# mad-red/VSR-guided-CIC

Measured on AMD Instinct MI355X. Metric: decoded tokens/sec at batch=100, beam=5, 36x2048 regions, higher is better.
Workload: dtype f16x2; 1 GPU; beam-5 decode, batch 100 images/GPU, 36 regions x 2048-d, 10 slots, seq_len 20, vocab 10000 (BASELINE configs[2]); beam=5, batch_per_gpu=100, seq_len=20, parallelism=images sharded, dp1, no data-path collective, rccl_world_size_observed=1, collective_backend=nccl

## Files before the change

### vsr-guided-cic_amd/csrc/kernels.h

```cpp
#pragma once
#include <hip/hip_runtime.h>
#include <stdint.h>

namespace vsr {

constexpr int KMAX = 8;

__device__ __forceinline__ float slab_sum(const float* __restrict__ p, int nslab, long long stride, float init = 0.f) {
    float v[8];
#pragma unroll
    for (int k = 0; k < 8; ++k) v[k] = k < nslab ? p[k * stride] : 0.f;
    float s = init;
#pragma unroll
    for (int k = 0; k < 8; ++k)
        if (k < nslab) s += v[k];
    return s;
}

__device__ __forceinline__ float sigmoidf_(float x) { return 1.0f / (1.0f + expf(-x)); }

__device__ __forceinline__ uint16_t bf16_bits(float x) {
    typedef __bf16 b2 __attribute__((ext_vector_type(2)));
    typedef float f2 __attribute__((ext_vector_type(2)));
    const f2 v = {x, 0.f};
    return (uint16_t)(__builtin_bit_cast(uint32_t, __builtin_convertvector(v, b2)) & 0xffffu);
}
__device__ __forceinline__ uint2 bf16_bits4(float4 v) {
    typedef __bf16 b2 __attribute__((ext_vector_type(2)));
    typedef float f2 __attribute__((ext_vector_type(2)));
    const f2 lo = {v.x, v.y}, hi = {v.z, v.w};
    return make_uint2(__builtin_bit_cast(uint32_t, __builtin_convertvector(lo, b2)), __builtin_bit_cast(uint32_t, __builtin_convertvector(hi, b2)));
}

__device__ __forceinline__ void img_store(uint16_t* __restrict__ img, long long idx, float v, float isc) {
    if (isc == 0.f) { img[idx] = bf16_bits(v); return; }
    const float x = v * isc;
    const _Float16 hi = (_Float16)x;
    const _Float16 lo = (_Float16)(x - (float)hi);
    uint16_t* g = img + ((idx >> 3) << 4) + (idx & 7);
    g[0] = __builtin_bit_cast(uint16_t, hi);
    g[8] = __builtin_bit_cast(uint16_t, lo);
}
__device__ __forceinline__ void img_store4(uint16_t* __restrict__ img, long long idx , float4 v, float isc) {
    if (isc == 0.f) { *reinterpret_cast<uint2*>(img + idx) = bf16_bits4(v); return; }
    typedef _Float16 h4 __attribute__((ext_vector_type(4)));
    typedef float f4 __attribute__((ext_vector_type(4)));
    const f4 x = {v.x * isc, v.y * isc, v.z * isc, v.w * isc};
    const h4 hi = __builtin_convertvector(x, h4);
    const f4 rr = x - __builtin_convertvector(hi, f4);
    const h4 lo = __builtin_convertvector(rr, h4);
    uint16_t* g = img + ((idx >> 3) << 4) + (idx & 7);
    *reinterpret_cast<uint2*>(g) = __builtin_bit_cast(uint2, hi);
    *reinterpret_cast<uint2*>(g + 8) = __builtin_bit_cast(uint2, lo);
}

__device__ __forceinline__ float wave_sum(float v) {
#pragma unroll
    for (int o = 32; o > 0; o >>= 1) v += __shfl_xor(v, o, 64);
    return v;
}
__device__ __forceinline__ float wave_max(float v) {
#pragma unroll
    for (int o = 32; o > 0; o >>= 1) v = fmaxf(v, __shfl_xor(v, o, 64));
    return v;
}

__device__ __forceinline__ int xcd_item(int n) {
    const int chunk = (n + 7) >> 3;
    const int it = (blockIdx.x & 7) * chunk + (blockIdx.x >> 3);
    return it < n ? it : -1;
}

__global__ __launch_bounds__(256) void k_pool(const float* __restrict__ det, const int* __restrict__ row_img,
                                              const float* __restrict__ dmask, int R0, int D, float* __restrict__ vbar) {
    const int b = blockIdx.x, d = (blockIdx.y * 256 + threadIdx.x) * 4;
    const int img = row_img ? row_img[b] : b;
    const float* X = det + (long long)img * R0 * D;
    const float* mk = dmask + (long long)img * R0;
    float n = 0.f;
    for (int r = 0; r < R0; ++r) n += mk[r];
    if (d >= D) return;
    float4 s = make_float4(0.f, 0.f, 0.f, 0.f);
    for (int r = 0; r < R0; ++r) {
        const float4 v = *reinterpret_cast<const float4*>(X + (long long)r * D + d);
        s.x += v.x; s.y += v.y; s.z += v.z; s.w += v.w;
    }
    *reinterpret_cast<float4*>(vbar + (long long)b * D + d) = make_float4(s.x / n, s.y / n, s.z / n, s.w / n);
}

__global__ __launch_bounds__(256) void k_rowmask(const float* __restrict__ X, long long rows, int D, float* __restrict__ mask,
                                                 float* __restrict__ blockmax = nullptr) {
    const long long row = (long long)blockIdx.x * 4 + (threadIdx.x >> 6);
    const int lane = threadIdx.x & 63;
    float s = 0.f, mx = 0.f;
    if (row < rows) {
        for (int d = lane * 4; d < D; d += 256) {
            float4 v = *reinterpret_cast<const float4*>(X + row * D + d);
            s += (v.x + v.y) + (v.z + v.w);
            if (blockmax) mx = fmaxf(fmaxf(mx, fmaxf(fabsf(v.x), fabsf(v.y))), fmaxf(fabsf(v.z), fabsf(v.w)));
        }
        s = wave_sum(s);
        if (lane == 0) mask[row] = (s != 0.f) ? 1.f : 0.f;
    }
    if (blockmax) {
        __shared__ float wm[4];
        mx = wave_max(mx);
        if (lane == 0) wm[threadIdx.x >> 6] = mx;
        __syncthreads();
        if (threadIdx.x == 0) blockmax[blockIdx.x] = fmaxf(fmaxf(wm[0], wm[1]), fmaxf(wm[2], wm[3]));
    }
}
__global__ __launch_bounds__(1024) void k_max_reduce(const float* __restrict__ v, long long n, unsigned* __restrict__ out) {
    __shared__ float wm[16];
    float m = 0.f;
    bool nan = false;
    for (long long i = threadIdx.x; i < n; i += 1024) { const float x = v[i]; nan |= !(x == x); m = fmaxf(m, x); }
    if (nan) m = __int_as_float(0x7f800000);
    m = wave_max(m);
    if ((threadIdx.x & 63) == 0) wm[threadIdx.x >> 6] = m;
    __syncthreads();
    if (threadIdx.x == 0) {
        for (int w = 1; w < 16; ++w) m = fmaxf(m, wm[w]);
        *out = __float_as_uint(m);
    }
}

__global__ void k_index_rows(const int* __restrict__ slot_idx, const int* __restrict__ row_img, const float* __restrict__ bmask,
                             int B, int LR, int Rb, int n_img, int* __restrict__ ridx, float* __restrict__ rmask,
                             int* __restrict__ bad) {
    const long long i = (long long)blockIdx.x * blockDim.x + threadIdx.x;
    if (i >= (long long)B * LR) return;
    const int b = (int)(i / LR);
    const int img = row_img ? row_img[b] : b;
    const int id = slot_idx[i];
    int row = -1;
    if (id >= Rb || id < -1 || img < 0 || img >= n_img) atomicAdd(bad, 1);
    else if (id >= 0) row = img * Rb + id;
    ridx[i] = row;
    rmask[i] = row >= 0 ? bmask[row] : 0.f;
}

__global__ __launch_bounds__(64) void k_reorder_slots(const int* __restrict__ slot_in, const int* __restrict__ rank,
                                                      const float* __restrict__ verbs_in, const float* __restrict__ bmask,
                                                      const int* __restrict__ row_img, int L, int R, int Rb,
                                                      int* __restrict__ slot_out, float* __restrict__ verbs_out) {
    extern __shared__ int sh[];
    int* src = sh;
// ... 16 lines not shown
    }
    __syncthreads();
    for (int i = tid; i < L * R; i += 64) {
        const int j = i / R, r = i - j * R;
        slot_out[(long long)n * L * R + i] = src[j] >= 0 ? S[src[j] * R + r] : -1;
    }
    if (verbs_in)
        for (int j = tid; j < L; j += 64) {
            const int rk = rank[(long long)n * L + j];
            verbs_out[(long long)n * L + j] = (rk >= 0 && rk < L) ? verbs_in[(long long)n * L + rk] : -1.f;
        }
}

__global__ __launch_bounds__(256) void k_compact_count(const float* __restrict__ mask, int rows, int* __restrict__ bcount) {
    __shared__ int wsum[4];
    const int r = blockIdx.x * 256 + threadIdx.x;
    const bool v = r < rows && mask[r] != 0.f;
    const int n = __popcll(__ballot(v));
    if ((threadIdx.x & 63) == 0) wsum[threadIdx.x >> 6] = n;
    __syncthreads();
    if (threadIdx.x == 0) bcount[blockIdx.x] = wsum[0] + wsum[1] + wsum[2] + wsum[3];
}

__global__ __launch_bounds__(1024) void k_compact_scan(int* __restrict__ bcount, int nblocks, int* __restrict__ total) {
    __shared__ int part[1024];
    const int tid = threadIdx.x;
    const int per = (nblocks + 1023) / 1024;
    const int b0 = tid * per, b1 = min(nblocks, b0 + per);
    int n = 0;
    for (int b = b0; b < b1; ++b) n += bcount[b];
    part[tid] = n;
    __syncthreads();
    for (int o = 1; o < 1024; o <<= 1) {
        const int v = tid >= o ? part[tid - o] : 0;
        __syncthreads();
        part[tid] += v;
        __syncthreads();
    }
    int run = part[tid] - n;
    for (int b = b0; b < b1; ++b) { const int c = bcount[b]; bcount[b] = run; run += c; }
    if (tid == 1023) *total = part[1023];
}

__global__ __launch_bounds__(256) void k_compact_write(const float* __restrict__ mask, int rows, const int* __restrict__ boffset,
                                                       int* __restrict__ vlist) {
    __shared__ int wsum[4];
    const int r = blockIdx.x * 256 + threadIdx.x, lane = threadIdx.x & 63, wave = threadIdx.x >> 6;
    const bool v = r < rows && mask[r] != 0.f;
    const unsigned long long bal = __ballot(v);
    if (lane == 0) wsum[wave] = __popcll(bal);
    __syncthreads();
    int base = boffset[blockIdx.x];
    for (int w = 0; w < wave; ++w) base += wsum[w];
    if (v) vlist[base + __popcll(bal & ((1ull << lane) - 1ull))] = r;
}

__global__ void k_pad_row_list(int* __restrict__ vlist, int* __restrict__ counts, int bound) {
    const int i = blockIdx.x * blockDim.x + threadIdx.x;
    const int n = counts[0];
    if (i == 0) {
        if (n > bound) counts[3] = n - bound;
        if (counts[1] != 0) atomicAdd(counts + 2, counts[1]);
    }
    if (i >= n && i < bound) vlist[i] = n > 0 ? vlist[0] : 0;
}

__global__ void k_zero_rows_beyond(const int* __restrict__ vlist, const int* __restrict__ counts, int bound, int A, float* __restrict__ P) {
    const int n = counts[0];
    for (int i = bound + (int)blockIdx.x; i < n; i += (int)gridDim.x) {
        float* row = P + (long long)vlist[i] * A;
        for (int a = threadIdx.x; a < A; a += blockDim.x) row[a] = 0.f;
    }
}

__global__ void k_slab_reduce_scatter(const float* __restrict__ slabs, int nslab, long long stride, int rows, int A,
                                      const int* __restrict__ vlist, float* __restrict__ P, const int* __restrict__ rows_dev = nullptr) {
    const long long i = (long long)blockIdx.x * blockDim.x + threadIdx.x;
    if (rows_dev && *rows_dev < rows) rows = *rows_dev;
    if (i >= (long long)rows * A) return;
    const int m = (int)(i / A), a = (int)(i % A);
    float s = slab_sum(slabs + i, nslab, stride);
    P[(long long)vlist[m] * A + a] = s;
}

__global__ void k_vproj_finish(const float* __restrict__ slabs, int nsplit, long long stride, int B, int H,
                               const float* b_ih, const float* b_hh, const float* b_is, const float* b_hs,
                               const float* b_ig, const float* b_hg, float* __restrict__ out) {
    const long long i = (long long)blockIdx.x * blockDim.x + threadIdx.x;
    const int N = 6 * H;
    if (i >= (long long)B * N) return;
    const int n = (int)(i % N);
    float s = slab_sum(slabs + i, nsplit, stride);
    float bias;
    if (n < 4 * H) bias = b_ih[n] + b_hh[n];
    else if (n < 5 * H) bias = b_is[n - 4 * H] + b_hs[n - 4 * H];
    else bias = b_ig[n - 5 * H] + b_hg[n - 5 * H];
    out[i] = s + bias;
}

__global__ void k_slab_reduce(const float* __restrict__ slabs, int nsplit, long long stride, long long n, float* __restrict__ out) {
    const long long i = (long long)blockIdx.x * blockDim.x + threadIdx.x;
    if (i >= n) return;
    float s = slab_sum(slabs + i, nsplit, stride);
    out[i] = s;
}

__global__ void k_init_rows(int* __restrict__ slot, int* __restrict__ word, int bos, int n) {
    const int i = blockIdx.x * blockDim.x + threadIdx.x;
    if (i < n) { slot[i] = 0; word[i] = bos; }
}

__global__ void k_count_outside_unit(const float* __restrict__ x, long long n, int* __restrict__ count) {
    const long long i = (long long)blockIdx.x * blockDim.x + threadIdx.x;
    const bool bad = i < n && !(fabsf(x[i]) < 1.9990234375f);
    const unsigned long long b = __ballot(bad);
    if ((threadIdx.x & 63) == 0 && b) atomicAdd(count, __popcll(b));
}

__global__ void k_fill_i32(int* p, int v, int n) {
    const int i = blockIdx.x * blockDim.x + threadIdx.x;
    if (i < n) p[i] = v;
}
__global__ void k_i64_to_i32(const int64_t* src, long long src_stride, int* dst, int n, int hi, int* __restrict__ bad) {
    const int i = blockIdx.x * blockDim.x + threadIdx.x;
    if (i >= n) return;
    long long v = src[(long long)i * src_stride];
    if (v < 0 || v >= hi) {
        atomicAdd(bad, 1);
        v = v < 0 ? 0 : hi - 1;
    }
    dst[i] = (int)v;
}
__global__ void k_i32_to_i64(const int* src, int64_t* dst, int n) {
    const int i = blockIdx.x * blockDim.x + threadIdx.x;
    if (i < n) dst[i] = src[i];
}

__device__ __forceinline__ void lstm1_point(const float (&q)[6], float c_old, long long i, float* __restrict__ h1n, float* __restrict__ c1n,
                                            float* __restrict__ s_t, float* __restrict__ gpre, uint16_t* __restrict__ h1n16,
                                            uint16_t* __restrict__ s_t16, float isc) {
    const float c = sigmoidf_(q[1]) * c_old + sigmoidf_(q[0]) * tanhf(q[2]);
    const float tc = tanhf(c);
    const float h1v = sigmoidf_(q[3]) * tc, stv = sigmoidf_(q[4]) * tc;
    h1n[i] = h1v;
    c1n[i] = c;
    s_t[i] = stv;
    gpre[i] = q[5];
    if (h1n16) { img_store(h1n16, i, h1v, isc); img_store(s_t16, i, stv, isc); }
}

__global__ void k_lstm1(const float* __restrict__ pre, int nsplit, long long stride, const float* __restrict__ vproj,
                        int rpi, const int* __restrict__ parent, const float* __restrict__ c1_old, int M, int H,
                        float* __restrict__ h1n, float* __restrict__ c1n, float* __restrict__ s_t, float* __restrict__ gpre,
                        const float* __restrict__ xproj, const int* __restrict__ word, int nblk, int pre_by_parent,
                        uint16_t* __restrict__ h1n16, uint16_t* __restrict__ s_t16 , float isc = 0.f,
                        int skip5 = 0 ) {
    const long long i = (long long)blockIdx.x * blockDim.x + threadIdx.x;
    if (i >= (long long)M * H) return;
    const int row = (int)(i / H), j = (int)(i % H);
    const int prow = parent ? parent[row] : row;
    const long long base = (long long)(pre_by_parent ? prow : row) * 6 * H + j;
    const float* vp = vproj + (long long)(row / rpi) * 6 * H + j;
    const float* xp = xproj ? xproj + (long long)word[row] * 6 * H + j : nullptr;
    float q[6];
#pragma unroll
    for (int g = 0; g < 6; ++g) {
        const int sk = g == 5 ? skip5 : 0;
        float s = g < nblk ? slab_sum(pre + base + (long long)g * H + sk * stride, nsplit - sk, stride) : 0.f;
        if (xp) s += xp[(long long)g * H];
        q[g] = s + vp[(long long)g * H];
    }
// ... 834 lines not shown
            const float co = c1_old[(long long)(b * cb + wave) * H + j];
#pragma unroll
            for (int g = 0; g < 6; ++g) {
                const int sk = g == 5 ? skip5 : 0;
                sums[(wave * 7 + g) * SL_UB + u] = g < nblk ? slab_sum(pre + base + (long long)g * H + sk * stride, nsplit - sk, stride) : 0.f;
            }
            sums[(wave * 7 + 6) * SL_UB + u] = co;
        }
    }
    __syncthreads();
    if (wave == K || j >= H) return;
    const int pl = sel_s[wave], w = sel_s[KMAX + wave];
    const int row = b * K + wave;
    const float* xp = xproj + (long long)w * 6 * H + j;
    float q[6];
#pragma unroll
    for (int g = 0; g < 6; ++g) {
        float s = sums[(pl * 7 + g) * SL_UB + u];
        s += xp[(long long)g * H];
        q[g] = s + vp[g];
    }
    lstm1_point(q, sums[(pl * 7 + 6) * SL_UB + u], (long long)row * H + j, h1n, c1n, s_t, gpre, h1n16, s_t16, isc);
}

__global__ __launch_bounds__(64) void k_backtrack(int T, int B, int beam, int out_size, const float* __restrict__ seq,
                                                  const int* __restrict__ hist_parent, const int* __restrict__ hist_word,
                                                  const int* __restrict__ hist_gate, const float* __restrict__ hist_lpw,
                                                  const float* __restrict__ hist_lpg, int64_t* __restrict__ words, int64_t* __restrict__ gates,
                                                  float* __restrict__ lp_w, float* __restrict__ lp_g, float* __restrict__ scores) {
    extern __shared__ int bt[];
    const int b = blockIdx.x, lane = threadIdx.x;
    const int n = T * beam;
    int* par = bt;
    int* wrd = bt + n;
    int* gat = bt + 2 * n;
    for (int i = lane; i < n; i += 64) {
        const int t = i / beam, q = i - t * beam;
        const long long hrow = (long long)t * B * beam + b * beam + q;
        par[i] = hist_parent[hrow];
        wrd[i] = hist_word[hrow];
        gat[i] = hist_gate[hrow];
    }
    __shared__ int order[KMAX];
    if (lane == 0) {
        for (int q = 0; q < beam; ++q) order[q] = q;
        for (int a = 1; a < beam; ++a) {
// ... 29 lines not shown
```

### vsr-guided-cic_amd/csrc/vsrcap.hip

```cpp
#include "../../include/vsrcap.h"

#include <hip/hip_runtime.h>

#include <algorithm>
#include <cstdarg>
#include <cstdio>
#include <cstdlib>
#include <cstring>
#include <vector>

#include "gemm_route.h"
#include "step_gemms.h"
#include "kernels.h"
#include "train_kernels.h"

using namespace vsr;

static thread_local char g_err[512] = "";
static int fail(const char* fmt, ...) {
    va_list ap;
    va_start(ap, fmt);
    vsnprintf(g_err, sizeof(g_err), fmt, ap);
    va_end(ap);
    return 1;
// ... 380 lines not shown

static const size_t H2_HEAD = 4096;
constexpr int H2_NDYN = 512;
static_assert(H2_DYN0 * 4 + H2_NDYN * 4 <= 4096, "dynamic slots inside the head");
extern "C" size_t vsr_h2_weight_bytes(const vsr_handle* h) {
    if (!h) return 0;
    const float* p[B16_NW]; size_t n[B16_NW];
    vsr_weights none;
    memset(&none, 0, sizeof(none));
    b16_weight_list(h->d, none, p, n);
    size_t tot = H2_HEAD;
    for (int i = 0; i < B16_NW; ++i) tot += ((n[i] + 7) & ~size_t(7)) * sizeof(float);
    tot += (((size_t)h->d.vocab_size * h->d.input_encoding_size + 7) & ~size_t(7)) * sizeof(float);
    return tot + 256;
}
__global__ void k_h2_head_init(int* exps, unsigned* bounds, int* idx) {
    const int i = threadIdx.x;
    if (i < H2_NSLOT) {
        exps[i] = 0;
        bounds[i] = i == H2A_UNIT ? __float_as_uint(1.f) : 0u;
        idx[i] = i; idx[H2_NSLOT + i] = -1; idx[2 * H2_NSLOT + i] = i;
    }
}
__global__ void k_h2_prepare_exps(const unsigned* __restrict__ bounds, int R0, int* __restrict__ exps) {
    if (threadIdx.x != 0) return;
    const float r = __uint_as_float(bounds[H2A_REGION]), dt = __uint_as_float(bounds[H2A_DET]), sn = __uint_as_float(bounds[H2B_SENT]);
    exps[H2A_REGION] = h2_exp_of(r);
    exps[H2A_DET] = h2_exp_of(dt * (float)R0);
    exps[H2A_ATT] = h2_exp_of(fmaxf(r, sn));
}
extern "C" int vsr_refresh_h2_weights(vsr_handle* h, void* buffer, size_t bytes, void* stream) {
    if (!h) return fail("vsr_refresh_h2_weights: null handle");
    if (!buffer) {
        if (h->h2_on) void_derived(h, VOID_FLAVOUR);
        h->h2_on = false;
        h->h2.clear(); h->h2t.clear();
        return 0;
    }
    if (!h->bound) return fail("vsr_refresh_h2_weights: weights not bound");
    const vsr_dims& d = h->d;
    if (d.det_feat_size % 8 || d.input_encoding_size % 8 || d.rnn_size % 8 || d.att_size % 8)
        return fail("vsr_refresh_h2_weights: the f16x2 flavour needs det_feat_size, input_encoding_size, rnn_size and att_size to be "
                    "multiples of 8 (whole 8-element groups of the fp16-pair images); got %d %d %d %d", d.det_feat_size, d.input_encoding_size, d.rnn_size, d.att_size);
    if (bytes < vsr_h2_weight_bytes(h)) return fail("vsr_refresh_h2_weights: buffer too small");
    if (reinterpret_cast<uintptr_t>(buffer) & 255) return fail("vsr_refresh_h2_weights: buffer must be 256-byte aligned");
    hipStream_t s = (hipStream_t)stream;
    const float* p[B16_NW]; size_t n[B16_NW];
    b16_weight_list(h->d, h->w, p, n);
    char* base = reinterpret_cast<char*>(buffer);
// ... 99 lines not shown
    hipStream_t s = (hipStream_t)stream;
    const vsr_dims& d = h->d;
    const vsr_weights& w = h->w;
    const int H = d.rnn_size, A = d.att_size, D = d.det_feat_size, E = d.input_encoding_size;
    Ctx& c = h->c;
    c.B = B; c.R0 = R0; c.L = L; c.R = R; c.beam = beam; c.Mmax = B * beam;
    c.n_img = indexed ? n_img : 0; c.Rb = indexed ? Rb : 0;
    c.det = det; c.regions = regions;
    const size_t need = carve(h, c, reinterpret_cast<char*>(workspace));
    if (need > workspace_bytes) return fail("%s: workspace too small (%zu < %zu bytes)", who, workspace_bytes, need);
    c.ridx = c.ridx_buf;
    c.rows_are_images = indexed && row_img == nullptr && n_img == B;
    h->prepared = false;
    invalidate_train_ctx(h->tc);
    drop_saved_forwards_in(h->saved, workspace, need);
    h->ws_lo = reinterpret_cast<const char*>(workspace); h->ws_bytes = need;

    const long long rows = (long long)B * L * R;
    const long long prows = indexed ? (long long)n_img * Rb : rows;
    const bool h2b = h->h2_on;
    float* bm_regions = h2b ? c.scratch : nullptr;
    float* bm_det = h2b ? c.scratch + cdiv(prows, 4) : nullptr;
    if (h2b && (size_t)(cdiv(prows, 4) + cdiv((long long)(indexed ? n_img : B) * R0, 4)) > c.scratch_floats) return fail("%s: scratch too small for the operand bounds", who);
    hipLaunchKernelGGL(k_rowmask, dim3(cdiv(prows, 4)), dim3(256), 0, s, regions, prows, D, c.bmask, bm_regions);
    HIPCHK(hipMemsetAsync(c.nvalid_dev, 0, 4 * sizeof(int), s));
    if (indexed) {
        hipLaunchKernelGGL(k_index_rows, dim3(cdiv(rows, 256)), dim3(256), 0, s, slot_idx, row_img, c.bmask, B, L * R, Rb, n_img,
                           c.ridx_buf, c.rmask, c.nvalid_dev + 1);
    }
    {
        const int nb = (int)cdiv(prows, 256);
        hipLaunchKernelGGL(k_compact_count, dim3(nb), dim3(256), 0, s, c.bmask, (int)prows, c.bcount);
        hipLaunchKernelGGL(k_compact_scan, dim3(1), dim3(1024), 0, s, c.bcount, nb, c.nvalid_dev);
        hipLaunchKernelGGL(k_compact_write, dim3(nb), dim3(256), 0, s, c.bmask, (int)prows, c.bcount, c.vlist);
    }
    LAUNCHCHK();
    const long long bound = h->rows_bound > 0 ? std::min(h->rows_bound, prows) : 0;
    int* back = nullptr;
    if (bound > 0) {
        hipLaunchKernelGGL(k_pad_row_list, dim3(cdiv(bound, 256)), dim3(256), 0, s, c.vlist, c.nvalid_dev, (int)bound);
        LAUNCHCHK();
    } else {
        if (!h->host_back) HIPCHK(hipHostMalloc(reinterpret_cast<void**>(&h->host_back), 2 * sizeof(int), hipHostMallocDefault));
        back = h->host_back;
        HIPCHK(hipMemcpyAsync(back, c.nvalid_dev, 2 * sizeof(int), hipMemcpyDeviceToHost, s));
        if (!h->ev_count) HIPCHK(hipEventCreateWithFlags(&h->ev_count, hipEventDisableTiming));
        HIPCHK(hipEventRecord(h->ev_count, s));
    }

    const long long drows = (long long)(indexed ? n_img : B) * R0;
    hipLaunchKernelGGL(k_rowmask, dim3(cdiv(drows, 4)), dim3(256), 0, s, det, drows, D, c.dmask, bm_det);
    if (h2b) {
        hipLaunchKernelGGL(k_max_reduce, dim3(1), dim3(1024), 0, s, bm_regions, (long long)cdiv(prows, 4), h->h2_bounds + H2A_REGION);
        hipLaunchKernelGGL(k_max_reduce, dim3(1), dim3(1024), 0, s, bm_det, (long long)cdiv(drows, 4), h->h2_bounds + H2A_DET);
        hipLaunchKernelGGL(k_h2_prepare_exps, dim3(1), dim3(64), 0, s, h->h2_bounds, R0, h->h2_exps);
    }
    hipLaunchKernelGGL(k_pool, dim3(B, cdiv(D, 1024)), dim3(256), 0, s, det, indexed ? row_img : nullptr, c.dmask, R0, D, c.vbar);
    LAUNCHCHK();

    const int in1 = (d.h2_first_lstm ? H : 0) + D + E;
    const int voff = d.h2_first_lstm ? H : 0;
    {
        GemmBuilder g;
        GemmProb& p0 = g.prob(B, 4 * H, c.scratch, 6 * H);
        GemmBuilder::seg(p0, c.vbar, D, nullptr, w.lstm1_weight_ih + voff, in1, D, nullptr, H2A_DET);
        GemmProb& p1 = g.prob(B, H, c.scratch + 4 * H, 6 * H);
        GemmBuilder::seg(p1, c.vbar, D, nullptr, w.W1_is_weight + voff, in1, D, nullptr, H2A_DET);
        GemmProb& p2 = g.prob(B, H, c.scratch + 5 * H, 6 * H);
        GemmBuilder::seg(p2, c.vbar, D, nullptr, w.W1_ig_weight + voff, in1, D, nullptr, H2A_DET);
        const int ns = g.finish(h);
        const long long stride = (long long)B * 6 * H;
        for (int i = 0; i < 3; ++i) g.a.p[i].slab_stride = stride;
        if (g.launch(s, h)) return fail("vproj gemm launch failed");
        const long long n = (long long)B * 6 * H;
        hipLaunchKernelGGL(k_vproj_finish, dim3(cdiv(n, 256)), dim3(256), 0, s, c.scratch, ns, stride, B, H,
                           w.lstm1_bias_ih, w.lstm1_bias_hh, w.W1_is_bias, w.W1_hs_bias, w.W1_ig_bias, w.W1_hg_bias, c.vproj);
        LAUNCHCHK();
    }
    if (d.img_second_lstm) {
        const int in2 = H + 2 * D;
// ... 8 lines not shown
        LAUNCHCHK();
    }
    c.bounded = bound > 0;
    if (bound > 0) {
        c.nvalid = (int)bound;
        if (prows > bound)
            hipLaunchKernelGGL(k_zero_rows_beyond, dim3((unsigned)std::min<long long>(prows - bound, 2048)), dim3(128), 0, s, c.vlist, c.nvalid_dev, (int)bound, A, c.P);
    } else {
        HIPCHK(hipEventSynchronize(h->ev_count));
        c.nvalid = back[0];
        if (indexed && back[1] != 0) return fail("%s: %d slot entries index outside the feature bank [-1, %d) or name an image outside [0, %d)", who, back[1], Rb, n_img);
    }
    if (c.nvalid > 0) {
        GemmBuilder g;
        g.keep_fp32 = true;
        GemmProb& p0 = g.prob(c.nvalid, A, c.scratch, A);
        GemmBuilder::seg(p0, regions, D, c.vlist, w.att_va_weight, D, D, nullptr, H2A_REGION);
        const int ns = g.finish(h);
        const long long stride = (long long)c.nvalid * A;
        if ((size_t)stride * ns > c.scratch_floats)
            return fail("%s: att_va slabs (%lld x %d floats) exceed the workspace scratch (%zu)", who, stride, ns, c.scratch_floats);
        g.a.p[0].slab_stride = stride;
        if (g.launch(s, h)) return fail("att_va gemm launch failed");
        hipLaunchKernelGGL(k_slab_reduce_scatter, dim3(cdiv(stride, 256)), dim3(256), 0, s, c.scratch, ns, stride, c.nvalid, A, c.vlist, c.P,
                           bound > 0 ? c.nvalid_dev : (const int*)nullptr);
        LAUNCHCHK();
    }
    h->prepared = true;
    return 0;
}

extern "C" int vsr_prepare(vsr_handle* h, const float* det, int32_t B, int32_t R0, const float* regions, int32_t L,
                           int32_t R, int32_t beam, void* workspace, size_t workspace_bytes, void* stream) {
    return prepare_impl(h, det, B, R0, regions, 0, 0, nullptr, nullptr, L, R, beam, workspace, workspace_bytes, stream, "vsr_prepare");
}

extern "C" int vsr_prepare_indexed(vsr_handle* h, const float* det, int32_t n_img, int32_t R0, const float* bank, int32_t Rb,
                                   const int32_t* row_img, int32_t B, const int32_t* slot_idx, int32_t L, int32_t R,
                                   int32_t beam, void* workspace, size_t workspace_bytes, void* stream) {
    if (!slot_idx) return fail("vsr_prepare_indexed: null slot index list");
    return prepare_impl(h, det, B, R0, bank, n_img, Rb, row_img, slot_idx, L, R, beam, workspace, workspace_bytes, stream,
                        "vsr_prepare_indexed");
}

extern "C" int vsr_row_mask(const float* rows, int64_t n_rows, int32_t D, float* mask, void* stream) {
    if (!rows || !mask || n_rows <= 0 || D <= 0 || (D & 3)) return fail("vsr_row_mask: bad arguments");
    hipLaunchKernelGGL(k_rowmask, dim3(cdiv(n_rows, 4)), dim3(256), 0, (hipStream_t)stream, rows, (long long)n_rows, D, mask);
    LAUNCHCHK();
    return 0;
}

extern "C" int vsr_reorder_slots(const int32_t* slot_idx, const int32_t* rank, const float* verbs, const float* bank_mask,
                                 const int32_t* row_img, int32_t N, int32_t L, int32_t R, int32_t Rb, int32_t* slot_out,
                                 float* verbs_out, void* stream) {
    if (!slot_idx || !rank || !slot_out || N <= 0 || L <= 0 || R <= 0 || Rb <= 0) return fail("vsr_reorder_slots: bad arguments");
    if (verbs && !verbs_out) return fail("vsr_reorder_slots: verbs given without an output");
    hipLaunchKernelGGL(k_reorder_slots, dim3(N), dim3(64), (size_t)L * sizeof(int), (hipStream_t)stream, slot_idx, rank, verbs,
                       bank_mask, row_img, L, R, Rb, slot_out, verbs_out);
    LAUNCHCHK();
    return 0;
}

struct StepIO {
    int t = 0, M = 0, rpi = 1, cur = 0;
    const int* parent = nullptr;
    const int* word_prev = nullptr;
    const int* slot = nullptr;
    int fixed_slot = 0;
    int vmode = VM_TOPK, K = 1;
    float* full_out = nullptr; long long full_stride = 0;
// ... 48 lines not shown
    Ctx& c = h->c;
    const int H = d.rnn_size, A = d.att_size, V = d.vocab_size;
    const int M = io.M;
    float* const* so = c.st[io.cur];
    float* const* sn = c.st[io.cur ^ 1];
    float *c1o = so[1], *c2o = so[3];
    float *h1n = sn[0], *c1n = sn[1], *h2n = sn[2], *c2n = sn[3];
    const bool sh2 = h->h2_on && !h->bf16_on && h->x3_on && h->gk.h2_aimg;
    const bool sh = (h->bf16_on && h->bf16_a16) || sh2;
    const float isc = sh2 ? 32768.f : 0.f;
    const int* att_exp = sh2 ? h->h2_exps + H2A_ATT : nullptr;
    const bool sh_old = sh && c.st16_ok[io.cur];
    uint16_t *h1n16 = sh ? c.st16[io.cur ^ 1][0] : nullptr, *h2n16 = sh ? c.st16[io.cur ^ 1][1] : nullptr;
    uint16_t *s_t16 = sh ? c.s_t16 : nullptr, *g_t16 = sh ? c.g_t16 : nullptr, *att16 = sh ? c.att16 : nullptr;
    StepOperands o;
    o.M = M; o.parent = io.parent; o.x = w.embed_weight; o.word = io.word_prev;
    o.h1_old = so[0]; o.h2_old = so[2]; o.h1_new = h1n; o.h2_new = h2n; o.s_t = c.s_t; o.g_t = c.g_t; o.att = c.att;
    o.h1_old16 = sh_old ? c.st16[io.cur][0] : nullptr; o.h2_old16 = sh_old ? c.st16[io.cur][1] : nullptr;
    o.h1_new16 = h1n16; o.h2_new16 = h2n16; o.s_t16 = s_t16; o.g_t16 = g_t16; o.att16 = att16;
    const long long stride1 = (long long)M * 6 * H;

    if (io.s1_from_prev && io.sel_beam) {
        const SelBeamArgs& sb = *io.sel_beam;
        const int nslice = cdiv(H, SL_UB);
        with_const_1to8(sb.beam, [&](auto KK) {
            hipLaunchKernelGGL((k_select_lstm1<decltype(KK)::value>), dim3(sb.B * nslice), dim3((decltype(KK)::value + 1) * 64), 0, s, sb, c.pre1, c.pre1_ns, c.pre1_stride,
                               c.vproj, c1o, H, nslice, h1n, c1n, c.s_t, c.gpre, h->xproj, c.pre1_nblk, h1n16, s_t16, isc, c.pre1_skip5);
        });
    } else if (io.s1_from_prev && io.sel_simple) {
        hipLaunchKernelGGL(k_select_simple_lstm1, dim3(cdiv((long long)M * H, 256)), dim3(256), 0, s, *io.sel_simple, c.pre1, c.pre1_ns, c.pre1_stride,
                           c.vproj, c1o, M, H, h1n, c1n, c.s_t, c.gpre, h->xproj, c.pre1_nblk, h1n16, s_t16, isc, c.pre1_skip5, io.rpi);
    } else if (io.s1_from_prev) {
        hipLaunchKernelGGL(k_lstm1, dim3(cdiv((long long)M * H, 256)), dim3(256), 0, s, c.pre1, c.pre1_ns, c.pre1_stride, c.vproj, io.rpi,
                           io.parent, c1o, M, H, h1n, c1n, c.s_t, c.gpre, h->xproj, io.word_prev, c.pre1_nblk, 1, h1n16, s_t16, isc, c.pre1_skip5);
    } else {
        GemmBuilder g;
        const int nblk = add_lstm1(g, d, w, o, c.scratch, (io.t > 0 ? L1_H2 | L1_H1 : 0) | (h->xproj ? 0 : L1_X));
        int ns = 0;
        if (g.a.nprob > 0) {
            ns = g.finish(h);
            for (int i = 0; i < g.a.nprob; ++i) g.a.p[i].slab_stride = stride1;
            if (g.launch(s, h)) return fail("S1 gemm launch failed");
        }
        hipLaunchKernelGGL(k_lstm1, dim3(cdiv((long long)M * H, 256)), dim3(256), 0, s, c.scratch, ns, stride1, c.vproj, io.rpi,
                           io.parent, c1o, M, H, h1n, c1n, c.s_t, c.gpre, h->xproj, io.word_prev, nblk, 0, h1n16, s_t16, isc);
    }
    {
        GemmBuilder g;
        add_s2(g, d, w, o, c.scratch);
// ... 44 lines not shown
            g.a.p[i].C += c.pre1_skip5 * stride1; g.a.p[i].slab_stride = stride1; g.a.p[i].nslab = ns_pre1;
        }
        c.pre1_ns = (g.a.nprob > 1 ? ns_pre1 : ns6) + c.pre1_skip5; c.pre1_nblk = nblk6; c.pre1_stride = stride1;
        if (c.pre1_ns > 8) return fail("S6: the LSTM1 sums of the next step would need %d slabs (8 fit)", c.pre1_ns);
        const int ns_vocab = g.a.p[0].nslab = gemm_tight_slabs(g.a, 0);
        if (g.launch(s, h)) return fail("S6 gemm launch failed");
        launch_vocab(h, s, io, c.scratch, ns_vocab, stride, gate_args);
    }
    c.st16_ok[io.cur ^ 1] = sh;
    LAUNCHCHK();
    return 0;
}

static int check_ready(vsr_handle* h, const char* who) {
    if (!h) return fail("%s: null handle", who);
    if (!h->bound) return fail("%s: weights not bound", who);
    if (!h->prepared) return fail("%s: vsr_prepare() has not been called", who);
    return 0;
}

static int zero_state(vsr_handle* h, int M, hipStream_t s) {
    Ctx& c = h->c;
    const size_t n = (size_t)M * h->d.rnn_size * sizeof(float);
    HIPCHK(hipMemsetAsync(c.st[0][0], 0, (size_t)(reinterpret_cast<char*>(c.st[0][3]) - reinterpret_cast<char*>(c.st[0][0])) + n, s));
    HIPCHK(hipMemsetAsync(c.st16[0][0], 0, (size_t)M * h->d.rnn_size * 2 * sizeof(uint16_t), s));
    HIPCHK(hipMemsetAsync(c.st16[0][1], 0, (size_t)M * h->d.rnn_size * 2 * sizeof(uint16_t), s));
    c.st16_ok[0] = true;
    c.st16_ok[1] = false;
    hipLaunchKernelGGL(k_init_rows, dim3(cdiv(M, 256)), dim3(256), 0, s, c.slot[0], c.word[0], h->d.bos_idx, M);
    LAUNCHCHK();
    return 0;
}

extern "C" int vsr_bad_ids(vsr_handle* h, int32_t* count, void* stream) {
    if (!h || !count) return fail("vsr_bad_ids: null argument");
    if (!h->prepared) { *count = 0; return 0; }
    hipStream_t s = (hipStream_t)stream;
    int v[2] = {0, 0};
    HIPCHK(hipMemcpyAsync(v, h->c.nvalid_dev + 2, 2 * sizeof(int), hipMemcpyDeviceToHost, s));
    HIPCHK(hipStreamSynchronize(s));
    HIPCHK(hipMemsetAsync(h->c.nvalid_dev + 2, 0, 2 * sizeof(int), s));
    *count = v[0] + v[1];
    return 0;
}

static int decode_simple(vsr_handle* h, int vmode, uint64_t seed, const int64_t* forced_w, const int64_t* forced_g,
                         const float* verbs, int gt, int64_t* words, int64_t* gates, float* lp_w, float* lp_g, hipStream_t s, int rpi = 1) {
    Ctx& c = h->c;
    const int B = c.B * rpi, T = h->d.seq_len;
    if (verbs && vmode != VM_TOPK) return fail("verb forcing is only defined for greedy / beam decoding");
    if (zero_state(h, B, s)) return 1;
    if (vmode == VM_FORCED) {
// ... 169 lines not shown
```

Measured before the change: 413,800 tokens/s.

## Fuse setup kernels and vectorize select-LSTM1, pool and slab reduce

Several prologue launches are merged: the two row-mask passes run in one grid that also clears the counters, the max-reduce kernels are folded into the exponent-prep kernel, the compact scan is folded into the compact write, and the state memsets plus row init become one zero-state kernel. Separately, k_pool batches its row loads and uses smaller blocks, the slab reduce-scatter processes float4s, and a two-column select+LSTM1 kernel is added that is used when the pointers are aligned. The aim is fewer launches and better memory-level parallelism in per-step kernels. In exchange, compact_write now re-sums bcount prefixes redundantly in every block, and the float4 reduce-scatter assumes A is divisible by 4.

```diff
diff --git a/vsr-guided-cic_amd/csrc/kernels.h b/vsr-guided-cic_amd/csrc/kernels.h
--- a/vsr-guided-cic_amd/csrc/kernels.h
+++ b/vsr-guided-cic_amd/csrc/kernels.h
@@ -14,6 +14,27 @@
 #pragma unroll
     for (int k = 0; k < 8; ++k)
         if (k < nslab) s += v[k];
+    return s;
+}
+
+__device__ __forceinline__ float2 slab_sum2(const float* __restrict__ p, int nslab, long long stride) {
+    float2 v[8];
+#pragma unroll
+    for (int k = 0; k < 8; ++k) v[k] = k < nslab ? *reinterpret_cast<const float2*>(p + k * stride) : make_float2(0.f, 0.f);
+    float2 s = make_float2(0.f, 0.f);
+#pragma unroll
+    for (int k = 0; k < 8; ++k)
+        if (k < nslab) { s.x += v[k].x; s.y += v[k].y; }
+    return s;
+}
+__device__ __forceinline__ float4 slab_sum4(const float* __restrict__ p, int nslab, long long stride) {
+    float4 v[8];
+#pragma unroll
+    for (int k = 0; k < 8; ++k) v[k] = k < nslab ? *reinterpret_cast<const float4*>(p + k * stride) : make_float4(0.f, 0.f, 0.f, 0.f);
+    float4 s = make_float4(0.f, 0.f, 0.f, 0.f);
+#pragma unroll
+    for (int k = 0; k < 8; ++k)
+        if (k < nslab) { s.x += v[k].x; s.y += v[k].y; s.z += v[k].z; s.w += v[k].w; }
     return s;
 }
 
@@ -40,6 +61,15 @@
     uint16_t* g = img + ((idx >> 3) << 4) + (idx & 7);
     g[0] = __builtin_bit_cast(uint16_t, hi);
     g[8] = __builtin_bit_cast(uint16_t, lo);
+}
+__device__ __forceinline__ void img_store2(uint16_t* __restrict__ img, long long idx , float v0, float v1, float isc) {
+    if (isc == 0.f) { *reinterpret_cast<uint32_t*>(img + idx) = (uint32_t)bf16_bits(v0) | ((uint32_t)bf16_bits(v1) << 16); return; }
+    const float x0 = v0 * isc, x1 = v1 * isc;
+    const _Float16 hi0 = (_Float16)x0, hi1 = (_Float16)x1;
+    const _Float16 lo0 = (_Float16)(x0 - (float)hi0), lo1 = (_Float16)(x1 - (float)hi1);
+    uint16_t* g = img + ((idx >> 3) << 4) + (idx & 7);
+    *reinterpret_cast<uint32_t*>(g) = (uint32_t)__builtin_bit_cast(uint16_t, hi0) | ((uint32_t)__builtin_bit_cast(uint16_t, hi1) << 16);
+    *reinterpret_cast<uint32_t*>(g + 8) = (uint32_t)__builtin_bit_cast(uint16_t, lo0) | ((uint32_t)__builtin_bit_cast(uint16_t, lo1) << 16);
 }
 __device__ __forceinline__ void img_store4(uint16_t* __restrict__ img, long long idx , float4 v, float isc) {
     if (isc == 0.f) { *reinterpret_cast<uint2*>(img + idx) = bf16_bits4(v); return; }
@@ -73,7 +103,7 @@
 
 __global__ __launch_bounds__(256) void k_pool(const float* __restrict__ det, const int* __restrict__ row_img,
                                               const float* __restrict__ dmask, int R0, int D, float* __restrict__ vbar) {
-    const int b = blockIdx.x, d = (blockIdx.y * 256 + threadIdx.x) * 4;
+    const int b = blockIdx.x, d = (blockIdx.y * blockDim.x + threadIdx.x) * 4;
     const int img = row_img ? row_img[b] : b;
     const float* X = det + (long long)img * R0 * D;
     const float* mk = dmask + (long long)img * R0;
@@ -81,17 +111,30 @@
     for (int r = 0; r < R0; ++r) n += mk[r];
     if (d >= D) return;
     float4 s = make_float4(0.f, 0.f, 0.f, 0.f);
-    for (int r = 0; r < R0; ++r) {
-        const float4 v = *reinterpret_cast<const float4*>(X + (long long)r * D + d);
-        s.x += v.x; s.y += v.y; s.z += v.z; s.w += v.w;
+    for (int r0 = 0; r0 < R0; r0 += 8) {
+        float4 v[8];
+#pragma unroll
+        for (int k = 0; k < 8; ++k)
+            if (r0 + k < R0) v[k] = *reinterpret_cast<const float4*>(X + (long long)(r0 + k) * D + d);
+#pragma unroll
+        for (int k = 0; k < 8; ++k)
+            if (r0 + k < R0) { s.x += v[k].x; s.y += v[k].y; s.z += v[k].z; s.w += v[k].w; }
     }
     *reinterpret_cast<float4*>(vbar + (long long)b * D + d) = make_float4(s.x / n, s.y / n, s.z / n, s.w / n);
 }
 
-__global__ __launch_bounds__(256) void k_rowmask(const float* __restrict__ X, long long rows, int D, float* __restrict__ mask,
-                                                 float* __restrict__ blockmax = nullptr) {
-    const long long row = (long long)blockIdx.x * 4 + (threadIdx.x >> 6);
+struct RowMaskArgs {
+    const float* X[2]; long long rows[2]; float* mask[2]; float* blockmax[2];
+    int nblk0; int* zero4;
+};
+__global__ __launch_bounds__(256) void k_rowmask(const RowMaskArgs a, int D) {
+    const int set = (int)blockIdx.x >= a.nblk0 ? 1 : 0;
+    const int blk = (int)blockIdx.x - (set ? a.nblk0 : 0);
+    const float* __restrict__ X = a.X[set];
+    float* __restrict__ blockmax = a.blockmax[set];
+    const long long rows = a.rows[set], row = (long long)blk * 4 + (threadIdx.x >> 6);
     const int lane = threadIdx.x & 63;
+    if (a.zero4 && blockIdx.x == 0 && threadIdx.x < 4) a.zero4[threadIdx.x] = 0;
     float s = 0.f, mx = 0.f;
     if (row < rows) {
         for (int d = lane * 4; d < D; d += 256) {
@@ -100,18 +143,17 @@
             if (blockmax) mx = fmaxf(fmaxf(mx, fmaxf(fabsf(v.x), fabsf(v.y))), fmaxf(fabsf(v.z), fabsf(v.w)));
         }
         s = wave_sum(s);
-        if (lane == 0) mask[row] = (s != 0.f) ? 1.f : 0.f;
+        if (lane == 0) a.mask[set][row] = (s != 0.f) ? 1.f : 0.f;
     }
     if (blockmax) {
         __shared__ float wm[4];
         mx = wave_max(mx);
         if (lane == 0) wm[threadIdx.x >> 6] = mx;
         __syncthreads();
-        if (threadIdx.x == 0) blockmax[blockIdx.x] = fmaxf(fmaxf(wm[0], wm[1]), fmaxf(wm[2], wm[3]));
-    }
-}
-__global__ __launch_bounds__(1024) void k_max_reduce(const float* __restrict__ v, long long n, unsigned* __restrict__ out) {
-    __shared__ float wm[16];
+        if (threadIdx.x == 0) blockmax[blk] = fmaxf(fmaxf(wm[0], wm[1]), fmaxf(wm[2], wm[3]));
+    }
+}
+__device__ __forceinline__ float block_max_1024(const float* __restrict__ v, long long n, float* wm ) {
     float m = 0.f;
     bool nan = false;
     for (long long i = threadIdx.x; i < n; i += 1024) { const float x = v[i]; nan |= !(x == x); m = fmaxf(m, x); }
@@ -119,10 +161,9 @@
     m = wave_max(m);
     if ((threadIdx.x & 63) == 0) wm[threadIdx.x >> 6] = m;
     __syncthreads();
-    if (threadIdx.x == 0) {
+    if (threadIdx.x == 0)
         for (int w = 1; w < 16; ++w) m = fmaxf(m, wm[w]);
-        *out = __float_as_uint(m);
-    }
+    return m;
 }
 
 __global__ void k_index_rows(const int* __restrict__ slot_idx, const int* __restrict__ row_img, const float* __restrict__ bmask,
@@ -185,35 +226,20 @@
     if (threadIdx.x == 0) bcount[blockIdx.x] = wsum[0] + wsum[1] + wsum[2] + wsum[3];
 }
 
-__global__ __launch_bounds__(1024) void k_compact_scan(int* __restrict__ bcount, int nblocks, int* __restrict__ total) {
-    __shared__ int part[1024];
-    const int tid = threadIdx.x;
-    const int per = (nblocks + 1023) / 1024;
-    const int b0 = tid * per, b1 = min(nblocks, b0 + per);
-    int n = 0;
-    for (int b = b0; b < b1; ++b) n += bcount[b];
-    part[tid] = n;
-    __syncthreads();
-    for (int o = 1; o < 1024; o <<= 1) {
-        const int v = tid >= o ? part[tid - o] : 0;
-        __syncthreads();
-        part[tid] += v;
-        __syncthreads();
-    }
-    int run = part[tid] - n;
-    for (int b = b0; b < b1; ++b) { const int c = bcount[b]; bcount[b] = run; run += c; }
-    if (tid == 1023) *total = part[1023];
-}
-
-__global__ __launch_bounds__(256) void k_compact_write(const float* __restrict__ mask, int rows, const int* __restrict__ boffset,
-                                                       int* __restrict__ vlist) {
-    __shared__ int wsum[4];
+__global__ __launch_bounds__(256) void k_compact_write(const float* __restrict__ mask, int rows, const int* __restrict__ bcount,
+                                                       int* __restrict__ vlist, int* __restrict__ total) {
+    __shared__ int wsum[4], wpre[4];
     const int r = blockIdx.x * 256 + threadIdx.x, lane = threadIdx.x & 63, wave = threadIdx.x >> 6;
     const bool v = r < rows && mask[r] != 0.f;
     const unsigned long long bal = __ballot(v);
-    if (lane == 0) wsum[wave] = __popcll(bal);
-    __syncthreads();
-    int base = boffset[blockIdx.x];
+    int pre = 0;
+    for (int b = threadIdx.x; b < (int)blockIdx.x; b += 256) pre += bcount[b];
+#pragma unroll
+    for (int o = 32; o > 0; o >>= 1) pre += __shfl_xor(pre, o, 64);
+    if (lane == 0) { wsum[wave] = __popcll(bal); wpre[wave] = pre; }
+    __syncthreads();
+    int base = wpre[0] + wpre[1] + wpre[2] + wpre[3];
+    if (blockIdx.x == gridDim.x - 1 && threadIdx.x == 0) *total = base + wsum[0] + wsum[1] + wsum[2] + wsum[3];
     for (int w = 0; w < wave; ++w) base += wsum[w];
     if (v) vlist[base + __popcll(bal & ((1ull << lane) - 1ull))] = r;
 }
@@ -238,12 +264,12 @@
 
 __global__ void k_slab_reduce_scatter(const float* __restrict__ slabs, int nslab, long long stride, int rows, int A,
                                       const int* __restrict__ vlist, float* __restrict__ P, const int* __restrict__ rows_dev = nullptr) {
-    const long long i = (long long)blockIdx.x * blockDim.x + threadIdx.x;
+    const long long i = ((long long)blockIdx.x * blockDim.x + threadIdx.x) * 4;
     if (rows_dev && *rows_dev < rows) rows = *rows_dev;
     if (i >= (long long)rows * A) return;
     const int m = (int)(i / A), a = (int)(i % A);
-    float s = slab_sum(slabs + i, nslab, stride);
-    P[(long long)vlist[m] * A + a] = s;
+    const float4 s = slab_sum4(slabs + i, nslab, stride);
+    *reinterpret_cast<float4*>(P + (long long)vlist[m] * A + a) = s;
 }
 
 __global__ void k_vproj_finish(const float* __restrict__ slabs, int nsplit, long long stride, int B, int H,
@@ -268,9 +294,19 @@
     out[i] = s;
 }
 
-__global__ void k_init_rows(int* __restrict__ slot, int* __restrict__ word, int bos, int n) {
-    const int i = blockIdx.x * blockDim.x + threadIdx.x;
-    if (i < n) { slot[i] = 0; word[i] = bos; }
+__global__ __launch_bounds__(256) void k_zero_state(uint32_t* __restrict__ st, size_t n_st, uint32_t* __restrict__ img0,
+                                                    uint32_t* __restrict__ img1, size_t n_img, int* __restrict__ slot,
+                                                    int* __restrict__ word, int bos, int n) {
+    const size_t i = (size_t)blockIdx.x * blockDim.x + threadIdx.x, nt = (size_t)gridDim.x * blockDim.x;
+    auto zero = [&](uint32_t* p, size_t nw) {
+        uint4* p4 = reinterpret_cast<uint4*>(p);
+        for (size_t k = i; k < (nw >> 2); k += nt) p4[k] = make_uint4(0u, 0u, 0u, 0u);
+        for (size_t k = (nw & ~size_t(3)) + i; k < nw; k += nt) p[k] = 0u;
+    };
+    zero(st, n_st);
+    zero(img0, n_img);
+    zero(img1, n_img);
+    for (size_t k = i; k < (size_t)n; k += nt) { slot[k] = 0; word[k] = bos; }
 }
 
 __global__ void k_count_outside_unit(const float* __restrict__ x, long long n, int* __restrict__ count) {
@@ -299,17 +335,34 @@
     if (i < n) dst[i] = src[i];
 }
 
+__device__ __forceinline__ void lstm1_cell(const float (&q)[6], float c_old, float& c, float& h1v, float& stv) {
+    c = sigmoidf_(q[1]) * c_old + sigmoidf_(q[0]) * tanhf(q[2]);
+    const float tc = tanhf(c);
+    h1v = sigmoidf_(q[3]) * tc;
+    stv = sigmoidf_(q[4]) * tc;
+}
 __device__ __forceinline__ void lstm1_point(const float (&q)[6], float c_old, long long i, float* __restrict__ h1n, float* __restrict__ c1n,
                                             float* __restrict__ s_t, float* __restrict__ gpre, uint16_t* __restrict__ h1n16,
                                             uint16_t* __restrict__ s_t16, float isc) {
-    const float c = sigmoidf_(q[1]) * c_old + sigmoidf_(q[0]) * tanhf(q[2]);
-    const float tc = tanhf(c);
-    const float h1v = sigmoidf_(q[3]) * tc, stv = sigmoidf_(q[4]) * tc;
+    float c, h1v, stv;
+    lstm1_cell(q, c_old, c, h1v, stv);
     h1n[i] = h1v;
     c1n[i] = c;
     s_t[i] = stv;
     gpre[i] = q[5];
     if (h1n16) { img_store(h1n16, i, h1v, isc); img_store(s_t16, i, stv, isc); }
+}
+__device__ __forceinline__ void lstm1_point2(const float (&qa)[6], const float (&qb)[6], float2 c_old, long long i, float* __restrict__ h1n,
+                                             float* __restrict__ c1n, float* __restrict__ s_t, float* __restrict__ gpre,
+                                             uint16_t* __restrict__ h1n16, uint16_t* __restrict__ s_t16, float isc) {
+    float ca, ha, sa, cb, hb, sb;
+    lstm1_cell(qa, c_old.x, ca, ha, sa);
+    lstm1_cell(qb, c_old.y, cb, hb, sb);
+    *reinterpret_cast<float2*>(h1n + i) = make_float2(ha, hb);
+    *reinterpret_cast<float2*>(c1n + i) = make_float2(ca, cb);
+    *reinterpret_cast<float2*>(s_t + i) = make_float2(sa, sb);
+    *reinterpret_cast<float2*>(gpre + i) = make_float2(qa[5], qb[5]);
+    if (h1n16) { img_store2(h1n16, i, ha, hb, isc); img_store2(s_t16, i, sa, sb, isc); }
 }
 
 __global__ void k_lstm1(const float* __restrict__ pre, int nsplit, long long stride, const float* __restrict__ vproj,
@@ -1190,6 +1243,51 @@
     }
     lstm1_point(q, sums[(pl * 7 + 6) * SL_UB + u], (long long)row * H + j, h1n, c1n, s_t, gpre, h1n16, s_t16, isc);
 }
+template <int K>
+__global__ __launch_bounds__((K + 1) * 64) void k_select_lstm1_x2(const SelBeamArgs sel, const float* __restrict__ pre, int nsplit, long long stride,
+                                                                  const float* __restrict__ vproj, const float* __restrict__ c1_old, int H, int nslice,
+                                                                  float* __restrict__ h1n, float* __restrict__ c1n, float* __restrict__ s_t,
+                                                                  float* __restrict__ gpre, const float* __restrict__ xproj, int nblk,
+                                                                  uint16_t* __restrict__ h1n16, uint16_t* __restrict__ s_t16, float isc, int skip5) {
+    __shared__ float2 sums[K * 7 * SL_UB];
+    __shared__ int sel_s[2 * KMAX];
+    const int b = blockIdx.x / nslice, slice = blockIdx.x % nslice;
+    const int wave = threadIdx.x >> 6, u = threadIdx.x & 63, cb = sel.cb;
+    const int j = (slice * SL_UB + u) * 2;
+    float2 vp[6];
+#pragma unroll
+    for (int g = 0; g < 6; ++g) vp[g] = make_float2(0.f, 0.f);
+    if (wave == K) {
+        select_beam_wave<K>(sel, b, u, slice == 0, sel_s);
+    } else if (j < H) {
+#pragma unroll
+        for (int g = 0; g < 6; ++g) vp[g] = *reinterpret_cast<const float2*>(vproj + (long long)b * 6 * H + (long long)g * H + j);
+        if (wave < cb) {
+            const long long base = (long long)(b * cb + wave) * 6 * H + j;
+            const float2 co = *reinterpret_cast<const float2*>(c1_old + (long long)(b * cb + wave) * H + j);
+#pragma unroll
+            for (int g = 0; g < 6; ++g) {
+                const int sk = g == 5 ? skip5 : 0;
+                sums[(wave * 7 + g) * SL_UB + u] = g < nblk ? slab_sum2(pre + base + (long long)g * H + sk * stride, nsplit - sk, stride) : make_float2(0.f, 0.f);
+            }
+            sums[(wave * 7 + 6) * SL_UB + u] = co;
+        }
+    }
+    __syncthreads();
+    if (wave == K || j >= H) return;
+    const int pl = sel_s[wave], w = sel_s[KMAX + wave];
+    const int row = b * K + wave;
+    const float* xp = xproj + (long long)w * 6 * H + j;
+    float qa[6], qb[6];
+#pragma unroll
+    for (int g = 0; g < 6; ++g) {
+        float2 s = sums[(pl * 7 + g) * SL_UB + u];
+        const float2 x = *reinterpret_cast<const float2*>(xp + (long long)g * H);
+        s.x += x.x; s.y += x.y;
+        qa[g] = s.x + vp[g].x; qb[g] = s.y + vp[g].y;
+    }
+    lstm1_point2(qa, qb, sums[(pl * 7 + 6) * SL_UB + u], (long long)row * H + j, h1n, c1n, s_t, gpre, h1n16, s_t16, isc);
+}
 
 __global__ __launch_bounds__(64) void k_backtrack(int T, int B, int beam, int out_size, const float* __restrict__ seq,
                                                   const int* __restrict__ hist_parent, const int* __restrict__ hist_word,
diff --git a/vsr-guided-cic_amd/csrc/vsrcap.hip b/vsr-guided-cic_amd/csrc/vsrcap.hip
--- a/vsr-guided-cic_amd/csrc/vsrcap.hip
+++ b/vsr-guided-cic_amd/csrc/vsrcap.hip
@@ -426,9 +426,14 @@
         idx[i] = i; idx[H2_NSLOT + i] = -1; idx[2 * H2_NSLOT + i] = i;
     }
 }
-__global__ void k_h2_prepare_exps(const unsigned* __restrict__ bounds, int R0, int* __restrict__ exps) {
+__global__ __launch_bounds__(1024) void k_h2_prepare_exps(const float* __restrict__ bm_regions, long long n_regions, const float* __restrict__ bm_det,
+                                                          long long n_det, unsigned* __restrict__ bounds, int R0, int* __restrict__ exps) {
+    __shared__ float wm[2][16];
+    const float r = block_max_1024(bm_regions, n_regions, wm[0]), dt = block_max_1024(bm_det, n_det, wm[1]);
     if (threadIdx.x != 0) return;
-    const float r = __uint_as_float(bounds[H2A_REGION]), dt = __uint_as_float(bounds[H2A_DET]), sn = __uint_as_float(bounds[H2B_SENT]);
+    bounds[H2A_REGION] = __float_as_uint(r);
+    bounds[H2A_DET] = __float_as_uint(dt);
+    const float sn = __uint_as_float(bounds[H2B_SENT]);
     exps[H2A_REGION] = h2_exp_of(r);
     exps[H2A_DET] = h2_exp_of(dt * (float)R0);
     exps[H2A_ATT] = h2_exp_of(fmaxf(r, sn));
@@ -574,8 +579,14 @@
     float* bm_regions = h2b ? c.scratch : nullptr;
     float* bm_det = h2b ? c.scratch + cdiv(prows, 4) : nullptr;
     if (h2b && (size_t)(cdiv(prows, 4) + cdiv((long long)(indexed ? n_img : B) * R0, 4)) > c.scratch_floats) return fail("%s: scratch too small for the operand bounds", who);
-    hipLaunchKernelGGL(k_rowmask, dim3(cdiv(prows, 4)), dim3(256), 0, s, regions, prows, D, c.bmask, bm_regions);
-    HIPCHK(hipMemsetAsync(c.nvalid_dev, 0, 4 * sizeof(int), s));
+    const long long drows = (long long)(indexed ? n_img : B) * R0;
+    {
+        RowMaskArgs a;
+        a.X[0] = regions; a.rows[0] = prows; a.mask[0] = c.bmask; a.blockmax[0] = bm_regions;
+        a.X[1] = det; a.rows[1] = drows; a.mask[1] = c.dmask; a.blockmax[1] = bm_det;
+        a.nblk0 = (int)cdiv(prows, 4); a.zero4 = c.nvalid_dev;
+        hipLaunchKernelGGL(k_rowmask, dim3(cdiv(prows, 4) + cdiv(drows, 4)), dim3(256), 0, s, a, D);
+    }
     if (indexed) {
         hipLaunchKernelGGL(k_index_rows, dim3(cdiv(rows, 256)), dim3(256), 0, s, slot_idx, row_img, c.bmask, B, L * R, Rb, n_img,
                            c.ridx_buf, c.rmask, c.nvalid_dev + 1);
@@ -583,8 +594,7 @@
     {
         const int nb = (int)cdiv(prows, 256);
         hipLaunchKernelGGL(k_compact_count, dim3(nb), dim3(256), 0, s, c.bmask, (int)prows, c.bcount);
-        hipLaunchKernelGGL(k_compact_scan, dim3(1), dim3(1024), 0, s, c.bcount, nb, c.nvalid_dev);
-        hipLaunchKernelGGL(k_compact_write, dim3(nb), dim3(256), 0, s, c.bmask, (int)prows, c.bcount, c.vlist);
+        hipLaunchKernelGGL(k_compact_write, dim3(nb), dim3(256), 0, s, c.bmask, (int)prows, c.bcount, c.vlist, c.nvalid_dev);
     }
     LAUNCHCHK();
     const long long bound = h->rows_bound > 0 ? std::min(h->rows_bound, prows) : 0;
@@ -600,14 +610,10 @@
         HIPCHK(hipEventRecord(h->ev_count, s));
     }
 
-    const long long drows = (long long)(indexed ? n_img : B) * R0;
-    hipLaunchKernelGGL(k_rowmask, dim3(cdiv(drows, 4)), dim3(256), 0, s, det, drows, D, c.dmask, bm_det);
-    if (h2b) {
-        hipLaunchKernelGGL(k_max_reduce, dim3(1), dim3(1024), 0, s, bm_regions, (long long)cdiv(prows, 4), h->h2_bounds + H2A_REGION);
-        hipLaunchKernelGGL(k_max_reduce, dim3(1), dim3(1024), 0, s, bm_det, (long long)cdiv(drows, 4), h->h2_bounds + H2A_DET);
-        hipLaunchKernelGGL(k_h2_prepare_exps, dim3(1), dim3(64), 0, s, h->h2_bounds, R0, h->h2_exps);
-    }
-    hipLaunchKernelGGL(k_pool, dim3(B, cdiv(D, 1024)), dim3(256), 0, s, det, indexed ? row_img : nullptr, c.dmask, R0, D, c.vbar);
+    if (h2b)
+        hipLaunchKernelGGL(k_h2_prepare_exps, dim3(1), dim3(1024), 0, s, bm_regions, (long long)cdiv(prows, 4), bm_det, (long long)cdiv(drows, 4),
+                           h->h2_bounds, R0, h->h2_exps);
+    hipLaunchKernelGGL(k_pool, dim3(B, cdiv(D, 256)), dim3(64), 0, s, det, indexed ? row_img : nullptr, c.dmask, R0, D, c.vbar);
     LAUNCHCHK();
 
     const int in1 = (d.h2_first_lstm ? H : 0) + D + E;
@@ -662,7 +668,7 @@
             return fail("%s: att_va slabs (%lld x %d floats) exceed the workspace scratch (%zu)", who, stride, ns, c.scratch_floats);
         g.a.p[0].slab_stride = stride;
         if (g.launch(s, h)) return fail("att_va gemm launch failed");
-        hipLaunchKernelGGL(k_slab_reduce_scatter, dim3(cdiv(stride, 256)), dim3(256), 0, s, c.scratch, ns, stride, c.nvalid, A, c.vlist, c.P,
+        hipLaunchKernelGGL(k_slab_reduce_scatter, dim3(cdiv(stride, 4 * 256)), dim3(256), 0, s, c.scratch, ns, stride, c.nvalid, A, c.vlist, c.P,
                            bound > 0 ? c.nvalid_dev : (const int*)nullptr);
         LAUNCHCHK();
     }
@@ -685,7 +691,10 @@
 
 extern "C" int vsr_row_mask(const float* rows, int64_t n_rows, int32_t D, float* mask, void* stream) {
     if (!rows || !mask || n_rows <= 0 || D <= 0 || (D & 3)) return fail("vsr_row_mask: bad arguments");
-    hipLaunchKernelGGL(k_rowmask, dim3(cdiv(n_rows, 4)), dim3(256), 0, (hipStream_t)stream, rows, (long long)n_rows, D, mask);
+    RowMaskArgs a;
+    memset(&a, 0, sizeof(a));
+    a.X[0] = rows; a.rows[0] = (long long)n_rows; a.mask[0] = mask; a.nblk0 = (int)cdiv(n_rows, 4);
+    hipLaunchKernelGGL(k_rowmask, dim3(cdiv(n_rows, 4)), dim3(256), 0, (hipStream_t)stream, a, D);
     LAUNCHCHK();
     return 0;
 }
@@ -780,9 +789,15 @@
 
     if (io.s1_from_prev && io.sel_beam) {
         const SelBeamArgs& sb = *io.sel_beam;
-        const int nslice = cdiv(H, SL_UB);
+        uintptr_t al = 0, al16 = reinterpret_cast<uintptr_t>(h1n16) | reinterpret_cast<uintptr_t>(s_t16);
+        for (const void* p : {(const void*)c.pre1, (const void*)c.vproj, (const void*)c1o, (const void*)h1n, (const void*)c1n, (const void*)c.s_t,
+                              (const void*)c.gpre, (const void*)h->xproj})
+            al |= reinterpret_cast<uintptr_t>(p);
+        const bool x2 = H % 2 == 0 && (al & 7) == 0 && (al16 & 3) == 0;
+        const int nslice = cdiv(H, x2 ? 2 * SL_UB : SL_UB);
         with_const_1to8(sb.beam, [&](auto KK) {
-            hipLaunchKernelGGL((k_select_lstm1<decltype(KK)::value>), dim3(sb.B * nslice), dim3((decltype(KK)::value + 1) * 64), 0, s, sb, c.pre1, c.pre1_ns, c.pre1_stride,
+            constexpr int K = decltype(KK)::value;
+            hipLaunchKernelGGL(x2 ? k_select_lstm1_x2<K> : k_select_lstm1<K>, dim3(sb.B * nslice), dim3((K + 1) * 64), 0, s, sb, c.pre1, c.pre1_ns, c.pre1_stride,
                                c.vproj, c1o, H, nslice, h1n, c1n, c.s_t, c.gpre, h->xproj, c.pre1_nblk, h1n16, s_t16, isc, c.pre1_skip5);
         });
     } else if (io.s1_from_prev && io.sel_simple) {
@@ -873,12 +888,12 @@
 static int zero_state(vsr_handle* h, int M, hipStream_t s) {
     Ctx& c = h->c;
     const size_t n = (size_t)M * h->d.rnn_size * sizeof(float);
-    HIPCHK(hipMemsetAsync(c.st[0][0], 0, (size_t)(reinterpret_cast<char*>(c.st[0][3]) - reinterpret_cast<char*>(c.st[0][0])) + n, s));
-    HIPCHK(hipMemsetAsync(c.st16[0][0], 0, (size_t)M * h->d.rnn_size * 2 * sizeof(uint16_t), s));
-    HIPCHK(hipMemsetAsync(c.st16[0][1], 0, (size_t)M * h->d.rnn_size * 2 * sizeof(uint16_t), s));
+    const size_t n_st = ((size_t)(reinterpret_cast<char*>(c.st[0][3]) - reinterpret_cast<char*>(c.st[0][0])) + n) / 4;
+    hipLaunchKernelGGL(k_zero_state, dim3((unsigned)std::min<size_t>(cdiv((long long)n_st, 4 * 256), 2048)), dim3(256), 0, s,
+                       reinterpret_cast<uint32_t*>(c.st[0][0]), n_st, reinterpret_cast<uint32_t*>(c.st16[0][0]),
+                       reinterpret_cast<uint32_t*>(c.st16[0][1]), n / 4, c.slot[0], c.word[0], h->d.bos_idx, M);
     c.st16_ok[0] = true;
     c.st16_ok[1] = false;
-    hipLaunchKernelGGL(k_init_rows, dim3(cdiv(M, 256)), dim3(256), 0, s, c.slot[0], c.word[0], h->d.bos_idx, M);
     LAUNCHCHK();
     return 0;
 }
```

Result: faster. 423,200 tokens/s (median of 6 runs) (+2.3%).
